# sloisel/MultiGridBarrier.jl

Measured on AMD Instinct MI355X. Metric: Newton iters/sec + wall-clock to converge, 2D P2 p-Laplace L=9, higher is better.
Workload: dtype f64

## Files before the change

### multigridbarrier.jl_amd/csrc/api.cpp

```cpp
#include <chrono>
#include <cmath>
#include <cstring>
#include <algorithm>
#include <limits>
#include <memory>
#include <string>

#include "interpolate.hpp"
#include "problem.hpp"

using namespace mgbhip;

mgbhip_problem* problem_create(mgbhip_ctx* ctx, const mgbhip_problem_desc* d, mgbhip_problem* share);
int core_run(mgbhip_problem* P, double* z, const double* c, const mgbhip_options* opt, mgbhip_core_result* res);
int matched_t_run(mgbhip_problem* P, const double* z, const double* c, double t_default, double* t_out);

#ifdef MGB_STEP_PROBE
namespace mgbhip { void mf_debug_probe(long long* out64); }
#endif

static thread_local std::string g_last_error;

struct DeviceGuard {
    int prev = -1, dev = -1;
// ... 165 lines not shown

int mgbhip_hessian_pattern(mgbhip_problem* P, int32_t level, int64_t* nnz, const int32_t** rowptr,
                           const int32_t** colidx) {
    MGB_API_BEGIN_ON(P)
    check_level(P, level);
    P->ensure_plan(level);
    if (nnz) *nnz = P->levels[level].nnz;
    if (rowptr) *rowptr = P->levels[level].hHptr.data();
    if (colidx) *colidx = P->levels[level].hHcol.data();
    return MGBHIP_OK;
    MGB_API_END
}

int mgbhip_solve(mgbhip_problem* P, int32_t level, const double* g, double* x) {
    MGB_API_BEGIN_ON(P)
    check_level(P, level);
    MGB_REQUIRE(g && x, "null argument");
    hipStream_t st = P->stream();
    const size_t m = (size_t)P->levels[level].m;
    P->d_g.upload(g, m, st);
    P->factor(level);
    P->trisolve(level, P->d_g.p, P->d_nv.p);
    int status = P->levels[level].solver.status(st);
    if (status != MGBHIP_OK && P->lu_fallback(level, P->d_g.p, P->d_nv.p)) status = MGBHIP_OK;
    P->d_nv.download(x, m, st);
    MGB_HIP_CHECK(hipStreamSynchronize(st));
    if (status != MGBHIP_OK) g_last_error = "Cholesky met a non-positive pivot";
    return status;
    MGB_API_END
}

int mgbhip_set_hessian(mgbhip_problem* P, int32_t level, const double* values) {
    MGB_API_BEGIN_ON(P)
    check_level(P, level);
    MGB_REQUIRE(values, "null argument");
    P->ensure_plan(level);
    mgbhip::Level& L = P->levels[level];
    MGB_REQUIRE(L.Hval.n >= (size_t)L.nnz, "this level keeps no CSR value array");
    L.Hval.upload(values, (size_t)L.nnz, P->stream());
    MGB_HIP_CHECK(hipStreamSynchronize(P->stream()));
    L.have_H = true;
    L.H_in_slab = false;
    L.factored = false;
    return MGBHIP_OK;
    MGB_API_END
}

int mgbhip_solve_newton(mgbhip_problem* P, int32_t level, const double* g, double* x, double* lambda2) {
    MGB_API_BEGIN_ON(P)
    check_level(P, level);
    MGB_REQUIRE(g && x, "null argument");
    hipStream_t st = P->stream();
    const size_t m = (size_t)P->levels[level].m;
    P->d_g.upload(g, m, st);
    P->factor(level, P->d_g.p);
    P->trisolve_carried(level, P->d_nv.p);
    int status = P->levels[level].solver.status(st);
    if (status != MGBHIP_OK && P->lu_fallback(level, P->d_g.p, P->d_nv.p)) status = MGBHIP_OK;
    P->d_nv.download(x, m, st);
    MGB_HIP_CHECK(hipStreamSynchronize(st));
    if (lambda2) {
        double acc = 0.0;
        for (size_t i = 0; i < m; ++i) acc += g[i] * x[i];
        *lambda2 = acc;
    }
    if (status != MGBHIP_OK) g_last_error = "Cholesky met a non-positive pivot";
    return status;
    MGB_API_END
}

int mgbhip_problem_set_sharding(mgbhip_problem* P, int32_t level, int64_t n_iface, const int32_t* iface_cols, const double* own_mask) {
    MGB_API_BEGIN_ON(P)
    check_level(P, level);
    mgbhip::Level& L = P->levels[level];
    MGB_REQUIRE(!L.solver.analyzed, "sharding must be set before the first solve of the level");
    MGB_REQUIRE(own_mask != nullptr && n_iface >= 0 && n_iface <= L.m && (n_iface == 0 || iface_cols), "bad sharding arguments");
    L.h_iface.assign(iface_cols, iface_cols + n_iface);
    for (int64_t i = 0; i < n_iface; ++i) {
        MGB_REQUIRE(L.h_iface[i] >= 0 && L.h_iface[i] < L.m, "interface column out of range");
        MGB_REQUIRE(i == 0 || L.h_iface[i] > L.h_iface[i - 1], "interface columns must be strictly increasing");
// ... 8 lines not shown

int mgbhip_problem_set_collective(mgbhip_problem* P, mgbhip_allreduce_fn fn, void* user, int32_t accepts_device_ptr) {
    MGB_API_BEGIN_ON(P)
    P->coll_fn = fn;
    P->coll_user = user;
    P->coll_device = accepts_device_ptr != 0;
    return MGBHIP_OK;
    MGB_API_END
}

int mgbhip_newton_direction(mgbhip_problem* P, int32_t level, const double* s, const double* c, const double* z0, double* x,
                            double* lambda2, int32_t* condensed) {
    MGB_API_BEGIN_ON(P)
    check_level(P, level);
    MGB_REQUIRE(s && c && z0 && x, "null argument");
    hipStream_t st = P->stream();
    const size_t m = (size_t)P->levels[level].m;
    stage_inputs(P, level, s, c, z0);
    P->eval_f1(level, P->d_x.p, P->d_z0.p, P->d_c.p, P->d_g.p);
    P->eval_f2(level, P->d_x.p, P->d_z0.p, P->d_c.p, false, P->d_g.p);
    if (condensed) *condensed = P->levels[level].H_condensed ? 1 : 0;
    P->factor(level, P->d_g.p);
    P->trisolve_carried(level, P->d_nv.p);
    const int status = P->levels[level].solver.status(st);
    P->d_nv.download(x, m, st);
    if (lambda2) {
        std::vector<double> g(m);
        P->d_g.download(g.data(), m, st);
        MGB_HIP_CHECK(hipStreamSynchronize(st));
        double acc = 0.0;
        for (size_t i = 0; i < m; ++i) acc += g[i] * x[i];
        *lambda2 = acc;
    }
    MGB_HIP_CHECK(hipStreamSynchronize(st));
    if (status != MGBHIP_OK) g_last_error = "Cholesky met a non-positive pivot";
    return status;
    MGB_API_END
}


static double* vec_scratch(mgbhip_ctx* c, int64_t len) {
    c->vscratch.ensure((size_t)reduce_scratch_doubles(len));
    c->vscal.ensure(8);
    return c->vscratch.p;
}
static void same_ctx(const mgbhip_vec* a, const mgbhip_vec* b) {
    MGB_REQUIRE(a && b, "null vector");
// ... 149 lines not shown
    P->touch();
    P->eval_f1(level, s->buf.p, z0->buf.p, c->buf.p, grad->buf.p);
    return MGBHIP_OK;
    MGB_API_END
}

int mgbhip_f2_d(mgbhip_problem* P, int32_t level, const mgbhip_vec* s, const mgbhip_vec* c, const mgbhip_vec* z0) {
    MGB_API_BEGIN_ON(P)
    check_closure_args(P, level, s, c, z0);
    P->touch();
    P->eval_f2(level, s->buf.p, z0->buf.p, c->buf.p);
    return MGBHIP_OK;
    MGB_API_END
}

int mgbhip_solve_d(mgbhip_problem* P, int32_t level, const mgbhip_vec* g, mgbhip_vec* x) {
    MGB_API_BEGIN_ON(P)
    check_level(P, level);
    MGB_REQUIRE(g && x && g->ctx == P->ctx && x->ctx == P->ctx, "bad vector");
    MGB_REQUIRE(g->len == P->levels[level].m && x->len == g->len, "solve: length mismatch");
    hipStream_t st = P->stream();
    P->factor(level);
    P->trisolve(level, g->buf.p, x->buf.p);
    const int status = P->levels[level].solver.status(st);
    if (status != MGBHIP_OK) g_last_error = "Cholesky met a non-positive pivot";
    return status;
    MGB_API_END
}

int mgbhip_prolong_add(mgbhip_problem* P, int32_t level, const mgbhip_vec* s, mgbhip_vec* z) {
    MGB_API_BEGIN_ON(P)
    check_level(P, level);
    MGB_REQUIRE(s && z && s->ctx == P->ctx && z->ctx == P->ctx, "bad vector");
    const Level& Lv = P->levels[level];
    MGB_REQUIRE(s->len == Lv.m && z->len == Lv.rows, "prolong_add: length mismatch");
    launch_csr_matvec(Lv.rows, Lv.Rptr.p, Lv.Rcol.p, Lv.Rval.p, s->buf.p, z->buf.p, true, false, P->stream());
    P->touch();
    return MGBHIP_OK;
    MGB_API_END
}

static int node_map(mgbhip_problem* P, const double* z, double* F, double* Dz, int mode) {
    MGB_REQUIRE(P && z && F, "null argument");
    hipStream_t st = P->stream();
    P->d_z0.upload(z, (size_t)P->nu * P->n, st);
    ElemParams E = P->base_params(-1, nullptr, P->d_z0.p, nullptr);
    if (Dz) {
// ... 168 lines not shown
```

### multigridbarrier.jl_amd/csrc/driver.cpp

```cpp
#include <chrono>
#include <cstdio>
#include <cstdlib>
#include <cmath>
#include <cstring>
#include <functional>
#include <limits>

#include "problem.hpp"

using namespace mgbhip;

namespace {

constexpr double EPS = std::numeric_limits<double>::epsilon();

bool debug_on() {
    static const bool on = [] { const char* e = getenv("MGBHIP_DEBUG"); return e && e[0] == '1'; }();
    return on;
}
#define DBG(...) do { if (debug_on()) { fprintf(stderr, __VA_ARGS__); } } while (0)

struct Stop {
    double lambda_tol;
    double theta;
// ... 162 lines not shown
    double y = C.F0(P->d_x.p);
    if (!std::isfinite(y)) throw InvalidArgument("newton: initial objective value is not finite");
    double ymin = y;
    if (P->sharded()) { P->d_gpart.ensure((size_t)C.m); P->d_gnpart.ensure((size_t)C.m); }
    C.F1(P->d_x.p, P->d_g.p, P->d_gpart.p);
    VecStats gs = vec_stats(P, C.level, P->d_g.p, C.m);
    if (gs.bad != 0.0 || !std::isfinite(gs.sumsq)) throw InvalidArgument("newton: initial gradient has non-finite entries");
    double gnorm = std::sqrt(gs.sumsq);
    double gmin = gnorm;
    double incmin = INFINITY;
    int k = 0;
    bool converged = false;
    Level& L = P->levels[C.level];
    struct RobustReset {
        MfSolver& s;
        ~RobustReset() { s.robust = false; }
    } robust_reset{L.solver};
    while (k < maxit && !converged) {
        ++k;
        C.F2(P->d_x.p);
        auto t0 = std::chrono::steady_clock::now();
        int fstatus = MGBHIP_OK;
        int leaf_flag = 0;
        for (int attempt = 0; attempt < 2; ++attempt) {
            P->factor(C.level, C.rhs_of_g());
            P->trisolve_carried(C.level, P->d_nv.p);
            const double seq = P->next_seq();
            launch_dir_finish(P->d_nv.p, P->d_g.p, C.m, P->d_scratch.p, P->d_scal.p, L.solver.status_flags_rw(), P->pin.dev, st,
                              P->own_mask(C.level), seq);
            L.solver.flags_cleared();
            P->wait_results(seq);
            P->pin.i[1] = P->pin.d[5] != 0.0 ? 1 : 0;
            leaf_flag |= P->pin.d[6] != 0.0 ? 1 : 0;
            P->pin.i[2] = leaf_flag;
            fstatus = MfSolver::status_from(P->pin.i + 1, L.solver.factored_condensed);
            if (P->sharded()) {
                P->pin.d[5] = fstatus != MGBHIP_OK ? 1.0 : 0.0;
                P->allreduce_host(P->pin.d + 2, 4, 0);
                fstatus = P->pin.d[5] != 0.0 ? MGBHIP_ERR_NOT_SPD : MGBHIP_OK;
            }
            const bool at_floor = std::fabs(P->pin.d[4]) <= EPS * std::fmax(std::fabs(y), 1.0);
            const bool suspicious = fstatus != MGBHIP_OK || P->pin.d[3] != 0.0 || !std::isfinite(P->pin.d[2]) ||
                                    (!(P->pin.d[4] > 0) && !at_floor);
            if (!suspicious || attempt == 1 || !L.solver.has_inverse_path() || L.solver.robust) break;
            DBG("newton[lev %d] k=%d: direction rejected (status %d, lambda^2=%.3e): refactoring with the substitution kernels\n",
                C.level, k, fstatus, P->pin.d[4]);
            L.solver.robust = true;
            L.factored = false;
        }
        if (fstatus != MGBHIP_OK && P->lu_fallback(C.level, P->d_g.p, P->d_nv.p)) {
            DBG("newton[lev %d] k=%d: LDL' met a zero pivot; direction from the pivoted LU fallback\n", C.level, k);
            launch_dir_finish(P->d_nv.p, P->d_g.p, C.m, P->d_scratch.p, P->d_scal.p, L.solver.status_flags_rw(), P->pin.dev, st,
                              P->own_mask(C.level));
            L.solver.flags_cleared();
            MGB_HIP_CHECK(hipStreamSynchronize(st));
            fstatus = MGBHIP_OK;
        }
// ... 231 lines not shown
    const bool sh = P->sharded();
    if (sh) { P->d_gpart.ensure((size_t)m); P->d_gnpart.ensure((size_t)m); }
    P->eval_f1(lev, P->d_x.p, P->d_z0.p, P->d_c.p, P->d_g.p, sh ? P->d_gpart.p : nullptr);
    P->eval_f1(lev, P->d_x.p, P->d_z0.p, P->d_c0.p, P->d_gn.p, sh ? P->d_gnpart.p : nullptr);
    launch_axpy(-1.0, P->d_g.p, P->d_gn.p, m, st);
    if (sh) launch_axpy(-1.0, P->d_gpart.p, P->d_gnpart.p, m, st);
    P->eval_f2(lev, P->d_x.p, P->d_z0.p, P->d_c0.p);
    if (sh) {
        P->d_tmp.ensure((size_t)m + 1);
        P->factor(lev, P->d_gpart.p);
        P->trisolve_carried(lev, P->d_tmp.p);
        int bad = P->levels[lev].solver.status(st) != MGBHIP_OK;
        MGB_HIP_CHECK(hipMemcpyAsync(P->d_nv.p, P->d_tmp.p, sizeof(double) * (size_t)m, hipMemcpyDeviceToDevice, st));
        P->levels[lev].factored = false;
        P->factor(lev, P->d_gnpart.p);
        P->trisolve_carried(lev, P->d_tmp.p);
        bad |= P->levels[lev].solver.status(st) != MGBHIP_OK;
        MGB_HIP_CHECK(hipMemcpyAsync(P->d_xn.p, P->d_tmp.p, sizeof(double) * (size_t)m, hipMemcpyDeviceToDevice, st));
        double fb = bad ? 1.0 : 0.0;
        P->allreduce_host(&fb, 1, 0);
        if (fb != 0.0) return MGBHIP_OK;
    } else {
        P->factor(lev);
        if (P->levels[lev].solver.status(st) != MGBHIP_OK) return MGBHIP_OK;
        P->trisolve(lev, P->d_g.p, P->d_nv.p);
        P->trisolve(lev, P->d_gn.p, P->d_xn.p);
    }
    const double d = dev_dot(P, lev, P->d_gn.p, P->d_xn.p, m);
    const double b = dev_dot(P, lev, P->d_g.p, P->d_xn.p, m) + dev_dot(P, lev, P->d_gn.p, P->d_nv.p, m);
    if (!(d > 0)) return MGBHIP_OK;
    const double tstar = -b / (2 * d);
    if (!(std::isfinite(tstar) && tstar > 0)) return MGBHIP_OK;
    *t_out = std::fmin(std::fmax(tstar, std::sqrt(EPS)), t_default);
    return MGBHIP_OK;
}
```

### multigridbarrier.jl_amd/csrc/mf_numeric.hip

```cpp
#include <hip/hip_runtime.h>

#include <cstdio>

#include <algorithm>
#include <cstdlib>

#include "../../include/mgbhip.h"
#include "mf_solver.hpp"

namespace mgbhip {

namespace {

#ifdef MGB_STEP_PROBE
__device__ long long g_probe[64];
#define SPL(i) do { if (threadIdx.x == 0 && gridDim.x == 1024 && blockIdx.x == 700 && j0 == 0) g_probe[48 + i] = wall_clock64(); } while (0)
#define SP(i) do { if (threadIdx.x == 0 && gridDim.x == 4096 && blockIdx.x == 3000) g_probe[40 + i] = wall_clock64(); if (threadIdx.x == 0 && gridDim.x == 1024 && blockIdx.x == 700) g_probe[24 + i] = wall_clock64(); } while (0)
#else
#define SPL(i) do { } while (0)
#define SP(i) do { } while (0)
#endif

typedef double double4_t __attribute__((ext_vector_type(4)));
constexpr int TX = 16;
// ... 1499 lines not shown
    PROBE(3);
    double4_t acc[4];
#pragma unroll
    for (int tb = 0; tb < 4; ++tb) acc[tb] = double4_t{0.0, 0.0, 0.0, 0.0};
#pragma unroll
    for (int kk = 0; kk < NB / 4; ++kk) {
        const double s = Pa[4 * kk + fk][16 * wave + fr16];
#pragma unroll
        for (int tb = 0; tb < 4; ++tb) {
            if (ti == tj && tb > wave) continue;
            acc[tb] = __builtin_amdgcn_mfma_f64_16x16x4f64(Pb[4 * kk + fk][16 * tb + fr16], s, acc[tb], 0, 0, 0);
        }
    }
    const int nskip = (blockIdx.x == 0 && look) ? nbn : 0;
#pragma unroll
    for (int tb = 0; tb < 4; ++tb)
#pragma unroll
        for (int r = 0; r < 4; ++r) {
            const int row = rbase + 16 * wave + fr16, col = cbase + 16 * tb + fk + 4 * r;
            if (row < m && col < m && row >= col && !(row - j1 < nskip && col - j1 < nskip))
                W[row + (int64_t)col * m] = cw[tb][r] - acc[tb][r];
        }
    PROBE(4);
}

__global__ __launch_bounds__(256) void mf_tri_pack(int m, const double* __restrict__ F, double* __restrict__ packed, int unpack,
                                                   double* __restrict__ Fout) {
    const int c = blockIdx.x;
    if (c >= m) return;
    const int64_t base = (int64_t)c * m - ((int64_t)c * (c - 1)) / 2;
    for (int r = c + threadIdx.x; r < m; r += 256) {
        if (unpack) Fout[r + (int64_t)c * m] = packed[base + (r - c)];
        else packed[base + (r - c)] = F[r + (int64_t)c * m];
    }
}

__global__ __launch_bounds__(256) void mf_big_diag0(const FrontDev* __restrict__ fr, int32_t first,
                                                    const double* __restrict__ arena, double* __restrict__ dscr,
                                                    int32_t* __restrict__ status) {
    __shared__ double Wv[NB][NB + 1];
    __shared__ double Dn[NB][NB + 1];
    __shared__ double Tm[16][17];
    __shared__ double dq[NB];
    const FrontDev F = fr[first + blockIdx.x];
    const int m = F.m, nb = min(NB, F.k), tid = threadIdx.x;
    const double* W = arena + F.F_off;
// ... 681 lines not shown
        d_a_dst.upload(ad, st);
        MGB_HIP_CHECK(hipStreamSynchronize(st));
        h_a_dst.swap(ad);
    }
    level_solves.assign(nlev, {});
    for (int32_t l = 0; l < nlev; ++l) {
        MfLaunch S{};
        for (auto& L : level_launches[l]) {
            if (!L.cls || L.tiny) { level_solves[l].push_back(L); continue; }
            if (S.count == 0) S = L;
            else {
                S.count += L.count;
                S.max_m = std::max(S.max_m, L.max_m);
                S.max_k = std::max(S.max_k, L.max_k);
            }
        }
        if (S.count) level_solves[l].insert(level_solves[l].begin(), S);
    }
    int32_t max_big = 1;
    for (auto& lev : level_launches)
        for (auto& L : lev)
            if (!L.cls) max_big = std::max(max_big, L.count);
    d_dscr.alloc((size_t)max_big * 2 * NB * NB);
    if (const char* e = getenv("MGBHIP_DEBUG"); e && atoi(e) >= 2) {
        fprintf(stderr, "[mgbhip] solver plan: n=%lld fronts=%d levels=%d arena=%.1f MB\n", (long long)plan.n, nf, nlev,
                plan.arena_doubles * 8e-6);
        for (int32_t l = 0; l < nlev; ++l)
            for (auto& L : level_launches[l]) {
                double sm = 0, sk = 0, fl = 0;
                for (int32_t q = L.first; q < L.first + L.count; ++q) {
                    const Front& f = plan.fronts[q];
                    sm += f.m; sk += f.k;
                    for (int c = 0; c < f.k; ++c) fl += (double)(f.m - c) * (f.m - c);
                }
                fprintf(stderr, "[mgbhip]   level %2d cls %3d count %7d max_m %4d max_k %4d avg_m %6.1f avg_k %6.1f Mflop %8.2f\n",
                        l, L.cls, L.count, L.max_m, L.max_k, sm / L.count, sk / L.count, fl * 1e-6);
            }
    }
    analyzed = true;
    MGB_HIP_CHECK(hipStreamSynchronize(st));
}


static StageTimers g_dummy_timers;
static StageTimers* timers_or_dummy(StageTimers* t, bool on) { return (t && on) ? t : &g_dummy_timers; }

bool MfSolver::launch_big_assemble(const MfLaunch& L, dim3 ga, const double* d_values, const int32_t* a_src_p, hipStream_t st,
                                   bool with_diag) {
    const size_t lds = (size_t)L.max_child * (size_t)L.max_m * sizeof(int32_t);
    if (L.max_child >= 1 && L.max_child <= GATHER_MAX_CHILD && lds <= 40 * 1024) {
        const int ct = CT;
        if (with_diag) ga.x += 1;
        hipLaunchKernelGGL(mf_big_gather, ga, dim3(256), lds, st, cur_fr, L.first, d_children.p, d_rel.p, a_src_p,
                           cur_adst, cur_acol, d_values, d_arena.p, L.max_m, d_dscr.p, d_status.p, with_diag ? 1 : 0, ct);
        return with_diag;
    } else
        hipLaunchKernelGGL(mf_big_assemble, ga, dim3(256), 0, st, cur_fr, L.first, d_children.p, d_rel.p, a_src_p,
                           cur_adst, cur_acol, d_values, d_arena.p);
    return false;
// ... 5 lines not shown
        const int64_t src = plan.a_src[t];
        const int64_t v = src < nnz ? (int64_t)value_map[src] : tail_base + (src - nnz);
        MGB_REQUIRE(v < (int64_t)INT32_MAX, "direct value index exceeds 32 bits");
        as[t] = (int32_t)v;
    }
    d_a_src_direct.upload(as, st);
    MGB_HIP_CHECK(hipStreamSynchronize(st));
}

void MfSolver::factor(const double* d_values, hipStream_t st, StageTimers* timers, bool direct, bool condensed) {
    MGB_REQUIRE(!direct || d_a_src_direct.n > 0, "MfSolver::factor: no direct value map");
    MGB_REQUIRE(!condensed || (direct && condensed_ok), "MfSolver::factor: condensed leaves are not enabled");
    const int32_t* a_src_p = condensed ? d_a_src_c.p : (direct ? d_a_src_direct.p : d_a_src.p);
    cur_fr = condensed ? d_fronts_c.p : d_fronts.p;
    cur_adst = condensed ? d_a_dst_c.p : d_a_dst.p;
    cur_acol = condensed ? d_a_colptr_c.p : d_a_colptr.p;
    MGB_REQUIRE(analyzed, "MfSolver::factor before analyze");
    if (timers) timers->begin("factor");
    factored_inv = !robust;
    if (!status_zero) MGB_HIP_CHECK(hipMemsetAsync(d_status.p, 0, sizeof(int32_t), st));
    status_zero = false;
    factored_condensed = condensed;
    static const bool lvl_timing = [] { const char* e = getenv("MGBHIP_LEVEL_TIMING"); return e && e[0] == '1'; }();
    int lvno = -1;
    for (auto& lev : level_launches) {
        ++lvno;
        char nm[32];
        snprintf(nm, sizeof(nm), "fac_lv%02d", lvno);
        StageScope lvscope(*timers_or_dummy(timers, lvl_timing), nm);
        for (auto& L : lev) {
            if (L.count == 0) continue;
            if (condensed && lvno == 0) continue;
            if (L.tiny) {
                hipLaunchKernelGGL(mf_factor_tiny, dim3((L.count + 15) / 16), dim3(256), 0, st, cur_fr, L.first,
                                   L.count, a_src_p, cur_adst, d_values, d_arena.p, d_status.p);
            } else if (L.wave) {
                const dim3 gw((L.count + 3) / 4);
                if (L.cls <= 32) {
                    const size_t lds = (size_t)4 * (32 * 33 / 2) * sizeof(double) + 4 * 64 * (sizeof(int64_t) + sizeof(int32_t));
                    hipLaunchKernelGGL(mf_factor_wave<32>, gw, dim3(256), lds, st, cur_fr, L.first, L.count, d_children.p, d_rel.p,
                                       a_src_p, cur_adst, d_values, d_arena.p, d_status.p);
                } else {
                    const size_t lds = (size_t)4 * (48 * 49 / 2) * sizeof(double) + 4 * 64 * (sizeof(int64_t) + sizeof(int32_t));
                    hipLaunchKernelGGL(mf_factor_wave<48>, gw, dim3(256), lds, st, cur_fr, L.first, L.count, d_children.p, d_rel.p,
                                       a_src_p, cur_adst, d_values, d_arena.p, d_status.p);
                }
// ... 21 lines not shown
                }
                if (L.inv && !robust) {
                    hipLaunchKernelGGL(mf_big_diag0, dim3(1), dim3(256), 0, st, cur_fr, L.first, d_arena.p, d_dscr.p, d_status.p);
                    for (int j0 = 0; j0 < L.max_k; j0 += NB) {
                        const int rem = L.max_m - j0;
                        const int T = std::max(0, (rem - 1 + ST - 1) / ST);
                        hipLaunchKernelGGL(mf_big_step, dim3(T * (T + 1) / 2 + 1, 1), dim3(256), 0, st, cur_fr, L.first, j0, d_arena.p,
                                           d_dscr.p, d_dvec.p, d_status.p, 0);
                    }
                } else {
                    for (int j0 = 0; j0 < L.max_k; j0 += NB) {
                        const int rem = L.max_m - j0;
                        hipLaunchKernelGGL(mf_big_panel, dim3(std::max(1, (rem - 1 + TR - 1) / TR), 1), dim3(256), 0, st, cur_fr,
                                           L.first, j0, d_arena.p, d_dscr.p, d_status.p, j0 == 0 ? 1 : 0);
                        const int T = (rem - 1 + ST - 1) / ST;
                        if (T > 0)
                            hipLaunchKernelGGL(mf_big_update, dim3(T * (T + 1) / 2 + 1, 1), dim3(256), 0, st, cur_fr, L.first, j0,
                                               d_arena.p, d_dscr.p, d_status.p);
                    }
                }
            } else if (L.inv && !robust) {
                const dim3 ga((L.max_m + CT - 1) / CT, L.count);
                const bool diag_done = launch_big_assemble(L, ga, d_values, a_src_p, st, true);
                const bool pre_diag = diag_done || L.count >= 24;
                if (pre_diag && !diag_done)
                    hipLaunchKernelGGL(mf_big_diag0, dim3(L.count), dim3(256), 0, st, cur_fr, L.first, d_arena.p, d_dscr.p,
                                       d_status.p);
                for (int j0 = 0; j0 < L.max_k; j0 += NB) {
                    const int rem = L.max_m - j0;
                    const int T = std::max(0, (rem - 1 + ST - 1) / ST);
                    const dim3 gs(T * (T + 1) / 2 + 1, L.count);
                    hipLaunchKernelGGL(mf_big_step, gs, dim3(256), 0, st, cur_fr, L.first, j0, d_arena.p, d_dscr.p,
                                       d_dvec.p, d_status.p, (j0 == 0 && !pre_diag) ? 1 : 0);
                }
            } else {
                const dim3 ga((L.max_m + CT - 1) / CT, L.count);
                launch_big_assemble(L, ga, d_values, a_src_p, st, false);
                for (int j0 = 0; j0 < L.max_k; j0 += NB) {
                    const int rem = L.max_m - j0;
                    const dim3 gp(std::max(1, (rem - 1 + TR - 1) / TR), L.count);
                    hipLaunchKernelGGL(mf_big_panel, gp, dim3(256), 0, st, cur_fr, L.first, j0, d_arena.p,
                                       d_dscr.p, d_status.p, j0 == 0 ? 1 : 0);
                    const int T = (rem - 1 + ST - 1) / ST;
                    if (T > 0) {
                        const dim3 gu(T * (T + 1) / 2 + 1, L.count);
                        hipLaunchKernelGGL(mf_big_update, gu, dim3(256), 0, st, cur_fr, L.first, j0, d_arena.p,
// ... 148 lines not shown
            for (int32_t q = L.first; q < L.first + L.count; ++q) {
                const Front& f = plan.fronts[q];
                const double mk = (double)(f.m - f.k), steps = (double)((f.k + NB - 1) / NB);
                extra += 2.0 * 0.5 * (mk * mk + mk * f.k) * std::max(0.0, steps - 1.0);
            }
        }
        if (lev_blocks) { big_levels += 1; blocks += lev_blocks; }
    }
    for (auto& lev : level_solves)
        for (auto& L : lev)
            if (L.count) bwd += 1;
    out[0] = blocks; out[1] = big_levels; out[2] = fac; out[3] = bwd;
    out[4] = (double)plan.arena_doubles; out[5] = (double)plan.factor_flops; out[6] = extra; out[7] = 0.0;
}

void MfSolver::status_async(int32_t* h_dst2, hipStream_t st) const {
    MGB_HIP_CHECK(hipMemcpyAsync(h_dst2, d_status.p, 2 * sizeof(int32_t), hipMemcpyDeviceToHost, st));
}

int MfSolver::status(hipStream_t st) {
    int32_t h[2] = {0, 0};
    d_status.download(h, 2, st);
    MGB_HIP_CHECK(hipStreamSynchronize(st));
    return status_from(h, factored_condensed);
}

bool MfSolver::enable_condensed(int64_t N, int P, const int32_t* ucol, int64_t slack0, int64_t nnz, int64_t tail_base,
                                hipStream_t st) {
    condensed_ok = false;
    int why = 0;
    struct Report { int& w; ~Report() { if (w) if (const char* e = getenv("MGBHIP_DEBUG"); e && atoi(e) >= 2) fprintf(stderr, "[mgbhip] condensed leaves: plan shape check %d failed\n", w); } } report{why};
    const int32_t nlev = (int32_t)plan.level_ptr.size() - 1;
    if (!analyzed || !plan.border || nlev < 2 || P > 7) { why = 1; return false; }
    const int32_t n0 = plan.level_ptr[1];
    if ((int64_t)n0 != N) { why = 2; return false; }
    const int32_t nbor = (int32_t)plan.n;
    std::vector<LeafDesc> desc((size_t)N);
    std::vector<char> seen((size_t)N, 0);
    for (int32_t i = 0; i < n0; ++i) {
        const Front& f = plan.fronts[i];
        const int32_t* idx = plan.front_idx.data() + f.idx_off;
        if (f.k != P + 1 || f.m > 15 || f.nchild != 0 || idx[f.m - 1] != nbor) { why = 3; return false; }
        const int64_t e = ((int64_t)idx[0] - slack0) / P;
        if (e < 0 || e >= N || seen[(size_t)e]) { why = 4; return false; }
        for (int q = 0; q < P; ++q)
            if ((int64_t)idx[q] != slack0 + e * P + q) { why = 5; return false; }
        if (idx[P] != ucol[e * P + (P - 1)] || idx[P] < 0) { why = 6; return false; }
// ... 53 lines not shown
```

### multigridbarrier.jl_amd/csrc/mf_solver.hpp

```cpp
#pragma once
#include <functional>

#include "common.hpp"
#include "mf_analysis.hpp"
#include "kernels.hpp"

namespace mgbhip {

struct FrontDev {
    int32_t k, m, nchild, a_cnt;
    int64_t F_off, idx_off, u_off, child_off, rel_off, a_off, acol_off;
    int64_t ug_off;
    int32_t packed;
    int32_t pad_;
};

struct MfLaunch {
    int32_t first, count;
    int32_t cls;
    int32_t max_m, max_k;
    int32_t max_child = 0;
    bool tiny = false;
    bool wave = false;
    bool inv = false;
    bool iface = false;
};

class MfSolver {
   public:
    MfPlan plan;
    void analyze(int64_t n, const int32_t* rowptr, const int32_t* colidx, hipStream_t st,
                 const double* coords = nullptr, int dim = 0, bool protect_peeled = false,
                 const int32_t* top = nullptr, int64_t ntop = 0);
    std::function<void(double*, int64_t)> iface_reduce;
    void factor(const double* d_values, hipStream_t st, StageTimers* timers, bool direct = false, bool condensed = false);
    bool enable_condensed(int64_t N, int P, const int32_t* ucol, int64_t slack0, int64_t nnz, int64_t tail_base, hipStream_t st);
    bool condensed_ready() const { return condensed_ok; }
    bool leaves_packed() const { return leaf_packed; }
    const LeafDesc* leaf_desc() const { return d_leaf_desc.p; }
    double* arena() { return d_arena.p; }
    int32_t* leaf_status() { return d_status.p + 1; }
    const int32_t* status_flags() const { return d_status.p; }
    int32_t* status_flags_rw() { return d_status.p; }
    void flags_cleared() { status_zero = true; leaf_zero = true; }
    bool leaf_flag_zero() const { return leaf_zero; }
    void leaf_flag_used() { leaf_zero = false; }
    void set_direct_map(const int32_t* value_map, int64_t nnz, int64_t tail_base, hipStream_t st);
    bool has_direct_map() const { return d_a_src_direct.n > 0; }
    void solve(const double* d_b, double* d_x, hipStream_t st, StageTimers* timers);
    void solve_border(double* d_x_np1, hipStream_t st, StageTimers* timers);
    void chain_stats(double* out8) const;
    int status(hipStream_t st);
    void status_async(int32_t* h_dst, hipStream_t st) const;
    static int status_from(const int32_t* flags2, bool with_leaves) {
        return (flags2[0] || (with_leaves && flags2[1])) ? MGBHIP_ERR_NOT_SPD : MGBHIP_OK;
    }
    bool factored_condensed = false;
    bool analyzed = false;
    bool robust = false;
    bool has_inverse_path() const { return uses_inv; }
    bool factored_inv = false;

   private:
    bool launch_big_assemble(const MfLaunch& L, dim3 grid, const double* d_values, const int32_t* a_src_p, hipStream_t st,
                             bool with_diag);
    void forward_pass(const double* d_b_np1, hipStream_t st, StageTimers* timers);
    void backward_pass(double* d_x_np1, hipStream_t st, StageTimers* timers);
    DevBuf<double> d_bx, d_xx, d_one;
    DevBuf<FrontDev> d_fronts;
    DevBuf<int32_t> d_front_idx, d_children, d_rel, d_a_src, d_a_src_direct, d_a_dst, d_a_colptr;
    DevBuf<int64_t> d_ug_ptr, d_ug_src;
    DevBuf<double> d_arena, d_uvec, d_y, d_tbig, d_tsol, d_dscr, d_dvec;
    DevBuf<double> d_ifpack;
    DevBuf<int32_t> d_status;
    bool condensed_ok = false;
    bool leaf_packed = false;
    std::vector<FrontDev> h_fronts;
    std::vector<int32_t> h_a_dst;
    DevBuf<FrontDev> d_fronts_c;
    DevBuf<int32_t> d_a_src_c, d_a_dst_c, d_a_colptr_c;
    DevBuf<LeafDesc> d_leaf_desc;
    const FrontDev* cur_fr = nullptr;
    const int32_t* cur_adst = nullptr;
    const int32_t* cur_acol = nullptr;
    std::vector<std::vector<MfLaunch>> level_launches;
    std::vector<std::vector<MfLaunch>> level_solves;
    int32_t lds_cap = 88;
    bool uses_inv = false;
    bool y_border_one = false;
    bool y_zero = false;
    bool status_zero = false, leaf_zero = false;
};

}
```

Baseline: 675.8.

## Fuse per-step big-front factor launches into one persistent level kernel with flag sync

Adds a persistent kernel that factors every big front in a tree level in a single launch. Lookahead workgroups produce the diagonal block inverses and tile workgroups apply the trailing updates, coordinated through epoch-tagged global flags with spin-waits. This removes the per-block-step kernel launches and the serialization between them. A timeout marks the factor as given up, and the caller then refactors with the old per-step launches, at the risk of deadlock-style stalls if the workgroups are not all co-resident, plus extra code complexity.

```diff
diff --git a/multigridbarrier.jl_amd/csrc/api.cpp b/multigridbarrier.jl_amd/csrc/api.cpp
--- a/multigridbarrier.jl_amd/csrc/api.cpp
+++ b/multigridbarrier.jl_amd/csrc/api.cpp
@@ -211,6 +211,11 @@
     P->factor(level);
     P->trisolve(level, P->d_g.p, P->d_nv.p);
     int status = P->levels[level].solver.status(st);
+    if (P->levels[level].solver.take_give_up()) {
+        P->factor(level);
+        P->trisolve(level, P->d_g.p, P->d_nv.p);
+        status = P->levels[level].solver.status(st);
+    }
     if (status != MGBHIP_OK && P->lu_fallback(level, P->d_g.p, P->d_nv.p)) status = MGBHIP_OK;
     P->d_nv.download(x, m, st);
     MGB_HIP_CHECK(hipStreamSynchronize(st));
@@ -245,6 +250,11 @@
     P->factor(level, P->d_g.p);
     P->trisolve_carried(level, P->d_nv.p);
     int status = P->levels[level].solver.status(st);
+    if (P->levels[level].solver.take_give_up()) {
+        P->factor(level, P->d_g.p);
+        P->trisolve_carried(level, P->d_nv.p);
+        status = P->levels[level].solver.status(st);
+    }
     if (status != MGBHIP_OK && P->lu_fallback(level, P->d_g.p, P->d_nv.p)) status = MGBHIP_OK;
     P->d_nv.download(x, m, st);
     MGB_HIP_CHECK(hipStreamSynchronize(st));
@@ -299,7 +309,12 @@
     if (condensed) *condensed = P->levels[level].H_condensed ? 1 : 0;
     P->factor(level, P->d_g.p);
     P->trisolve_carried(level, P->d_nv.p);
-    const int status = P->levels[level].solver.status(st);
+    int status = P->levels[level].solver.status(st);
+    if (P->levels[level].solver.take_give_up()) {
+        P->factor(level, P->d_g.p);
+        P->trisolve_carried(level, P->d_nv.p);
+        status = P->levels[level].solver.status(st);
+    }
     P->d_nv.download(x, m, st);
     if (lambda2) {
         std::vector<double> g(m);
@@ -495,7 +510,12 @@
     hipStream_t st = P->stream();
     P->factor(level);
     P->trisolve(level, g->buf.p, x->buf.p);
-    const int status = P->levels[level].solver.status(st);
+    int status = P->levels[level].solver.status(st);
+    if (P->levels[level].solver.take_give_up()) {
+        P->factor(level);
+        P->trisolve(level, g->buf.p, x->buf.p);
+        status = P->levels[level].solver.status(st);
+    }
     if (status != MGBHIP_OK) g_last_error = "Cholesky met a non-positive pivot";
     return status;
     MGB_API_END
diff --git a/multigridbarrier.jl_amd/csrc/driver.cpp b/multigridbarrier.jl_amd/csrc/driver.cpp
--- a/multigridbarrier.jl_amd/csrc/driver.cpp
+++ b/multigridbarrier.jl_amd/csrc/driver.cpp
@@ -208,6 +208,7 @@
         auto t0 = std::chrono::steady_clock::now();
         int fstatus = MGBHIP_OK;
         int leaf_flag = 0;
+        bool level_redo = false;
         for (int attempt = 0; attempt < 2; ++attempt) {
             P->factor(C.level, C.rhs_of_g());
             P->trisolve_carried(C.level, P->d_nv.p);
@@ -219,6 +220,14 @@
             P->pin.i[1] = P->pin.d[5] != 0.0 ? 1 : 0;
             leaf_flag |= P->pin.d[6] != 0.0 ? 1 : 0;
             P->pin.i[2] = leaf_flag;
+            if (!level_redo && L.solver.take_give_up((int32_t)P->pin.d[5])) {
+                DBG("newton[lev %d] k=%d: level kernel gave up a wait (%lld so far): refactoring with the per-step launches\n",
+                    C.level, k, (long long)L.solver.level_give_ups);
+                level_redo = true;
+                L.factored = false;
+                --attempt;
+                continue;
+            }
             fstatus = MfSolver::status_from(P->pin.i + 1, L.solver.factored_condensed);
             if (P->sharded()) {
                 P->pin.d[5] = fstatus != MGBHIP_OK ? 1.0 : 0.0;
@@ -496,7 +505,12 @@
         if (fb != 0.0) return MGBHIP_OK;
     } else {
         P->factor(lev);
-        if (P->levels[lev].solver.status(st) != MGBHIP_OK) return MGBHIP_OK;
+        int fst = P->levels[lev].solver.status(st);
+        if (P->levels[lev].solver.take_give_up()) {
+            P->factor(lev);
+            fst = P->levels[lev].solver.status(st);
+        }
+        if (fst != MGBHIP_OK) return MGBHIP_OK;
         P->trisolve(lev, P->d_g.p, P->d_nv.p);
         P->trisolve(lev, P->d_gn.p, P->d_xn.p);
     }
diff --git a/multigridbarrier.jl_amd/csrc/mf_numeric.hip b/multigridbarrier.jl_amd/csrc/mf_numeric.hip
--- a/multigridbarrier.jl_amd/csrc/mf_numeric.hip
+++ b/multigridbarrier.jl_amd/csrc/mf_numeric.hip
@@ -1545,6 +1545,309 @@
                 W[row + (int64_t)col * m] = cw[tb][r] - acc[tb][r];
         }
     PROBE(4);
+}
+
+typedef uint32_t __attribute__((address_space(1))) lv_gu32;
+typedef unsigned long long __attribute__((address_space(1))) lv_gu64;
+__device__ __forceinline__ double lv_ld(const double* p) {
+    return __longlong_as_double((long long)__hip_atomic_load((lv_gu64*)p, __ATOMIC_RELAXED, __HIP_MEMORY_SCOPE_AGENT));
+}
+__device__ __forceinline__ void lv_st(double* p, double v) {
+    __hip_atomic_store((lv_gu64*)p, (unsigned long long)__double_as_longlong(v), __ATOMIC_RELAXED, __HIP_MEMORY_SCOPE_AGENT);
+}
+
+struct LvFlags {
+    uint32_t* base;
+    int nblk, tm;
+    __device__ uint32_t* w(int b) const { return base + b; }
+    __device__ uint32_t* corner(int b) const { return base + nblk + b; }
+    __device__ uint32_t* col(int b, int I) const { return base + 2 * nblk + b * tm + I; }
+};
+
+__device__ __forceinline__ bool lv_acquire(uint32_t* const* fl, int n, uint32_t epoch, long long limit,
+                                           int32_t* status, int* s_ok, int tid) {
+    if (n == 0) return true;
+    if (tid < 64) {
+        bool ok = limit > 0;
+        const long long t0 = wall_clock64();
+        for (int i = 0; i < n && ok; ++i) {
+            while (__hip_atomic_load((lv_gu32*)fl[i], __ATOMIC_RELAXED, __HIP_MEMORY_SCOPE_AGENT) != epoch) {
+                if (wall_clock64() - t0 > limit) { ok = false; break; }
+                __builtin_amdgcn_s_sleep(1);
+            }
+        }
+        if (tid == 0) {
+            if (!ok) atomicOr(status, MF_LEVEL_GAVE_UP);
+            *s_ok = ok ? 1 : 0;
+        }
+    }
+    __syncthreads();
+    __builtin_amdgcn_fence(__ATOMIC_ACQUIRE, "wavefront");
+    const bool ok = *s_ok != 0;
+    __syncthreads();
+    return ok;
+}
+
+__device__ __forceinline__ void lv_publish(uint32_t* flag, uint32_t epoch, int tid) {
+    asm volatile("s_waitcnt vmcnt(0)" ::: "memory");
+    __syncthreads();
+    if (tid == 0) __hip_atomic_store((lv_gu32*)flag, epoch, __ATOMIC_RELAXED, __HIP_MEMORY_SCOPE_AGENT);
+}
+
+__device__ __forceinline__ void lv_write_mj(const double (*Wv)[NB + 1], const double* dq, double* W, double* dvec, int64_t idx_off,
+                                            int m, int j0, int nb, int lane, int wave) {
+    const int fr16 = lane & 15, fk = lane >> 4;
+    const int rt = wave & 1, ct = wave >> 1;
+    if (ct <= rt) {
+        double4_t accm = {0.0, 0.0, 0.0, 0.0};
+#pragma unroll
+        for (int kk = 0; kk < NB / 4; ++kk) {
+            const int kq = 4 * kk + fk;
+            accm = __builtin_amdgcn_mfma_f64_16x16x4f64(kq < nb ? Wv[kq][16 * ct + fr16] / dq[kq] : 0.0, Wv[kq][16 * rt + fr16], accm, 0, 0, 0);
+        }
+#pragma unroll
+        for (int r = 0; r < 4; ++r) {
+            const int row = 16 * rt + fr16, col = 16 * ct + fk + 4 * r;
+            if (row < nb && col < row) W[(j0 + col) + (int64_t)(j0 + row) * m] = accm[r];
+            else if (row < nb && col == row) dvec[idx_off + j0 + row] = accm[r];
+        }
+    }
+}
+
+__device__ __forceinline__ void lv_load_slot(const double* slot, double (*Wv)[NB + 1], double* dq, int nb, int tid) {
+    for (int i = tid; i < NB * NB; i += 256) {
+        const int rr = i % NB, c = i / NB;
+        const double v = (rr >= c && rr < nb) ? lv_ld(slot + rr + NB * c) : 0.0;
+        Wv[rr][c] = (rr > c) ? v : (rr == c ? 1.0 : 0.0);
+        if (rr == c) dq[rr] = (rr < nb) ? v : 1.0;
+    }
+}
+
+constexpr int LV_WAVES_PER_SIMD = 2;
+
+__global__ __launch_bounds__(256, LV_WAVES_PER_SIMD) void mf_big_step_level(
+        const FrontDev* __restrict__ fr, int32_t first, int32_t count, const int32_t* __restrict__ tile_pref,
+        double* __restrict__ arena, const double* __restrict__ dscr, double* __restrict__ lslot, double* __restrict__ dvec,
+        int32_t* __restrict__ status, uint32_t* __restrict__ flags, int nblkmax, int tmmax, uint32_t epoch, long long limit) {
+    __shared__ double Wv[NB][NB + 1];
+    __shared__ double Dn[NB][NB + 1];
+    __shared__ double Tm[16][17];
+    __shared__ double dq[NB], rdq[NB];
+    __shared__ double Pa[NB][ST + 1];
+    __shared__ double Pb[NB][ST + 1];
+    __shared__ int s_ok;
+    const int tid = threadIdx.x, lane = tid & 63, wave = tid >> 6;
+    const int fr16 = lane & 15, fk = lane >> 4;
+    const bool is_la = (int)blockIdx.x < count;
+    int f = 0, lin = 0;
+    if (is_la) {
+        f = blockIdx.x;
+    } else {
+        const int t = blockIdx.x - count;
+        while (f + 1 < count && tile_pref[f + 1] <= t) ++f;
+        lin = t - tile_pref[f];
+    }
+    const FrontDev F = fr[first + f];
+    const int m = F.m, k = F.k;
+    const int nblk = (k + NB - 1) / NB, Tmf = (m + ST - 1) / ST;
+    double* W = arena + F.F_off;
+    const LvFlags FL{flags + (int64_t)f * nblkmax * (2 + tmmax), nblkmax, tmmax};
+    double* myslots = lslot + (int64_t)f * nblkmax * (NB * NB);
+    const double* slot0 = dscr + (int64_t)f * 2 * (NB * NB);
+    uint32_t* wl[3];
+
+    if (is_la) {
+        lv_load_slot(slot0, Wv, dq, min(NB, k), tid);
+        for (int j = 0; j < nblk; ++j) {
+            const int j0 = j * NB, nb = min(NB, k - j0), j1 = j0 + nb;
+            const bool look = j1 < k;
+            const int nbn = look ? min(NB, k - j1) : 0;
+            __syncthreads();
+            if (tid < NB) rdq[tid] = 1.0 / dq[tid];
+            if ((j + 1) / 2 >= Tmf) lv_write_mj(Wv, dq, W, dvec, F.idx_off, m, j0, nb, lane, wave);
+            if (!look) break;
+            int nw = 0;
+            if (j >= 1) wl[nw++] = FL.col(j, (j + 1) / 2);
+            if (j + 1 >= 2) wl[nw++] = FL.corner(j + 1);
+            if (!lv_acquire(wl, nw, epoch, limit, status, &s_ok, tid)) return;
+            double pa[NB * ST / 256], cc[4];
+#pragma unroll
+            for (int u = 0; u < NB * ST / 256; ++u) {
+                const int i = tid + 256 * u, rr = i % ST, q = i / ST;
+                pa[u] = (q < nb && rr < nbn) ? lv_ld(W + (j1 + rr) + (int64_t)(j0 + q) * m) : 0.0;
+            }
+#pragma unroll
+            for (int t = 0; t < 4; ++t) {
+                const int i = tid + 256 * t, rr = i % NB, c = i / NB;
+                cc[t] = (rr >= c && rr < nbn) ? lv_ld(W + (j1 + rr) + (int64_t)(j1 + c) * m) : 0.0;
+            }
+#pragma unroll
+            for (int u = 0; u < NB * ST / 256; ++u) {
+                const int i = tid + 256 * u, rr = i % ST, q = i / ST;
+                Pa[q][rr] = pa[u];
+                Pb[q][rr] = 0.0;
+            }
+            __syncthreads();
+            if (wave < 2) slice_transform(Pa, Pa, Pb, Wv, rdq, lane, wave);
+            __syncthreads();
+            {
+                const int rt = wave & 1, ct = wave >> 1;
+                double4_t accd = {0.0, 0.0, 0.0, 0.0};
+#pragma unroll
+                for (int kk = 0; kk < NB / 4; ++kk)
+                    accd = __builtin_amdgcn_mfma_f64_16x16x4f64(Pb[4 * kk + fk][16 * ct + fr16], Pa[4 * kk + fk][16 * rt + fr16],
+                                                                accd, 0, 0, 0);
+#pragma unroll
+                for (int r = 0; r < 4; ++r) {
+                    const int rr = 16 * rt + fr16, c = 16 * ct + fk + 4 * r;
+                    Dn[rr][c] = -accd[r];
+                }
+            }
+            __syncthreads();
+#pragma unroll
+            for (int t = 0; t < 4; ++t) {
+                const int i = tid + 256 * t, rr = i % NB, c = i / NB;
+                Dn[rr][c] = (rr >= c && rr < nbn) ? cc[t] + Dn[rr][c] : 0.0;
+            }
+            __syncthreads();
+            block_ldlt32(Dn, dq, nbn, tid, status);
+            block_inverse32_sel(Dn, Wv, Tm, tid);
+            double* nslot = myslots + (int64_t)(j + 1) * (NB * NB);
+            for (int i = tid; i < NB * NB; i += 256) {
+                const int rr = i % NB, c = i / NB;
+                if (rr >= c && rr < nbn) lv_st(nslot + rr + NB * c, (rr == c) ? dq[rr] : Wv[rr][c]);
+            }
+            lv_publish(FL.w(j + 1), epoch, tid);
+            for (int i = tid; i < NB * NB; i += 256) {
+                const int rr = i % NB, c = i / NB;
+                if (rr == c) {
+                    if (rr >= nbn) dq[rr] = 1.0;
+                    Wv[rr][c] = 1.0;
+                } else if (rr < c || rr >= nbn) {
+                    Wv[rr][c] = 0.0;
+                }
+            }
+        }
+        return;
+    }
+
+    int I = (int)((sqrt(8.0 * lin + 1.0) - 1.0) * 0.5);
+    while ((I + 1) * (I + 2) / 2 <= lin) ++I;
+    while (I * (I + 1) / 2 > lin) --I;
+    const int J = lin - I * (I + 1) / 2;
+    const int r0 = ST * I, c0 = ST * J;
+    double cw[4][4];
+#pragma unroll
+    for (int tb = 0; tb < 4; ++tb)
+#pragma unroll
+        for (int r = 0; r < 4; ++r) {
+            const int row = r0 + 16 * wave + fr16, col = c0 + 16 * tb + fk + 4 * r;
+            cw[tb][r] = (row < m && col < m && row >= col) ? W[row + (int64_t)col * m] : 0.0;
+        }
+    const int jlast = min(2 * J + 1, nblk - 1);
+    for (int j = 0; j <= jlast; ++j) {
+        const int j0 = j * NB, nb = min(NB, k - j0), j1 = j0 + nb;
+        const bool mw = I == J && (j + 1) / 2 == J;
+        const bool work = c0 + ST - 1 >= j1 && m > j1;
+        if (!work && !mw) continue;
+        if (j >= 1) {
+            int nw = 0;
+            wl[nw++] = FL.w(j);
+            wl[nw++] = FL.col(j, I);
+            if (I != J) wl[nw++] = FL.col(j, J);
+            if (!lv_acquire(wl, nw, epoch, limit, status, &s_ok, tid)) return;
+        }
+        double pa[NB * ST / 256], pb[NB * ST / 256];
+#pragma unroll
+        for (int u = 0; u < NB * ST / 256; ++u) {
+            const int i = tid + 256 * u, rr = i % ST, q = i / ST;
+            const int r = r0 + rr, c = c0 + rr;
+            pa[u] = (q < nb && r >= j1 && r < m) ? lv_ld(W + r + (int64_t)(j0 + q) * m) : 0.0;
+            pb[u] = (I != J && q < nb && c >= j1 && c < m) ? lv_ld(W + c + (int64_t)(j0 + q) * m) : 0.0;
+        }
+        lv_load_slot(j == 0 ? slot0 : myslots + (int64_t)j * (NB * NB), Wv, dq, nb, tid);
+#pragma unroll
+        for (int u = 0; u < NB * ST / 256; ++u) {
+            const int i = tid + 256 * u, rr = i % ST, q = i / ST;
+            Pa[q][rr] = pa[u];
+            Pb[q][rr] = pb[u];
+        }
+        __syncthreads();
+        if (tid < NB) rdq[tid] = 1.0 / dq[tid];
+        if (mw) lv_write_mj(Wv, dq, W, dvec, F.idx_off, m, j0, nb, lane, wave);
+        __syncthreads();
+        if (work) {
+            if (I == J) {
+                slice_transform(Pa, Pa, Pb, Wv, rdq, lane, wave);
+            } else {
+                slice_transform(Pa, Pa, nullptr, Wv, rdq, lane, wave);
+                const int rr = 16 * wave + fr16;
+                double4_t acc0 = {0.0, 0.0, 0.0, 0.0}, acc1 = {0.0, 0.0, 0.0, 0.0};
+#pragma unroll
+                for (int kk = 0; kk < NB / 4; ++kk) {
+                    const double a = Pb[4 * kk + fk][rr];
+                    if (kk < 4) acc0 = __builtin_amdgcn_mfma_f64_16x16x4f64(Wv[fr16][4 * kk + fk], a, acc0, 0, 0, 0);
+                    acc1 = __builtin_amdgcn_mfma_f64_16x16x4f64(Wv[16 + fr16][4 * kk + fk], a, acc1, 0, 0, 0);
+                }
+#pragma unroll
+                for (int r = 0; r < 4; ++r) {
+                    const int q0 = fk + 4 * r, q1 = 16 + fk + 4 * r;
+                    Pb[q0][rr] = acc0[r] * rdq[q0];
+                    Pb[q1][rr] = acc1[r] * rdq[q1];
+                }
+            }
+            __syncthreads();
+            double4_t acc[4];
+#pragma unroll
+            for (int tb = 0; tb < 4; ++tb) acc[tb] = double4_t{0.0, 0.0, 0.0, 0.0};
+#pragma unroll
+            for (int kk = 0; kk < NB / 4; ++kk) {
+                const double s = Pa[4 * kk + fk][16 * wave + fr16];
+#pragma unroll
+                for (int tb = 0; tb < 4; ++tb) {
+                    if (I == J && tb > wave) continue;
+                    acc[tb] = __builtin_amdgcn_mfma_f64_16x16x4f64(Pb[4 * kk + fk][16 * tb + fr16], s, acc[tb], 0, 0, 0);
+                }
+            }
+#pragma unroll
+            for (int tb = 0; tb < 4; ++tb)
+#pragma unroll
+                for (int r = 0; r < 4; ++r) {
+                    const int row = r0 + 16 * wave + fr16, col = c0 + 16 * tb + fk + 4 * r;
+                    if (row >= j1 && col >= j1 && row < m && col < m && row >= col) cw[tb][r] = cw[tb][r] - acc[tb][r];
+                }
+        }
+        __syncthreads();
+        const bool pc = I == J && j + 2 < nblk && (j + 2) / 2 == J;
+        const bool pp = j + 1 < nblk && (j + 1) / 2 == J;
+        if (pc || pp) {
+            const int cb0 = (j + 2) * NB, cnb = pc ? min(NB, k - cb0) : 0;
+            const int pb0 = (j + 1) * NB, pnb = pp ? min(NB, k - pb0) : 0;
+#pragma unroll
+            for (int tb = 0; tb < 4; ++tb)
+#pragma unroll
+                for (int r = 0; r < 4; ++r) {
+                    const int row = r0 + 16 * wave + fr16, col = c0 + 16 * tb + fk + 4 * r;
+                    const bool sc = row >= col && row >= cb0 && row < cb0 + cnb && col >= cb0 && col < cb0 + cnb;
+                    const bool sp = pp && col >= pb0 && col < pb0 + NB && row < m && col < m && row >= col &&
+                                    !(row >= pb0 && row < pb0 + pnb && col < pb0 + pnb);
+                    if (sc || sp) lv_st(W + row + (int64_t)col * m, cw[tb][r]);
+                }
+            asm volatile("s_waitcnt vmcnt(0)" ::: "memory");
+            __syncthreads();
+            if (tid == 0) {
+                if (pc) __hip_atomic_store((lv_gu32*)FL.corner(j + 2), epoch, __ATOMIC_RELAXED, __HIP_MEMORY_SCOPE_AGENT);
+                if (pp) __hip_atomic_store((lv_gu32*)FL.col(j + 1, I), epoch, __ATOMIC_RELAXED, __HIP_MEMORY_SCOPE_AGENT);
+            }
+        }
+    }
+#pragma unroll
+    for (int tb = 0; tb < 4; ++tb)
+#pragma unroll
+        for (int r = 0; r < 4; ++r) {
+            const int row = r0 + 16 * wave + fr16, col = c0 + 16 * tb + fk + 4 * r;
+            if (col >= k && row < m && col < m && row >= col) W[row + (int64_t)col * m] = cw[tb][r];
+        }
 }
 
 __global__ __launch_bounds__(256) void mf_tri_pack(int m, const double* __restrict__ F, double* __restrict__ packed, int unpack,
@@ -2272,6 +2575,47 @@
         for (auto& L : lev)
             if (!L.cls) max_big = std::max(max_big, L.count);
     d_dscr.alloc((size_t)max_big * 2 * NB * NB);
+    {
+        static const int lv_cap = [] {
+            constexpr int blocks_per_cu = LV_WAVES_PER_SIMD;
+            int dev = 0, cus = 256;
+            if (hipGetDevice(&dev) == hipSuccess) (void)hipDeviceGetAttribute(&cus, hipDeviceAttributeMultiprocessorCount, dev);
+            return std::max(1, cus) * (blocks_per_cu - 1);
+        }();
+        std::vector<int32_t> pref;
+        int64_t nflags = 0, nslot = 0;
+        for (auto& lev : level_launches)
+            for (auto& L : lev) {
+                L.lv_wgs = 0;
+                if (L.cls || L.tiny || L.wave || L.iface || !L.inv || L.count == 0) continue;
+                const size_t lds = (size_t)L.max_child * (size_t)L.max_m * sizeof(int32_t);
+                if (!(L.max_child >= 1 && L.max_child <= GATHER_MAX_CHILD && lds <= 40 * 1024)) continue;
+                int64_t wgs = L.count, nblk = 0, tm = 0;
+                std::vector<int32_t> p(1, 0);
+                for (int32_t q = L.first; q < L.first + L.count; ++q) {
+                    const Front& f = plan.fronts[q];
+                    const int64_t t = (f.m + ST - 1) / ST;
+                    wgs += t * (t + 1) / 2;
+                    p.push_back(p.back() + (int32_t)(t * (t + 1) / 2));
+                    nblk = std::max<int64_t>(nblk, (f.k + NB - 1) / NB);
+                    tm = std::max(tm, t);
+                }
+                if (wgs > lv_cap || nblk < 2) continue;
+                L.lv_wgs = (int32_t)wgs;
+                L.lv_pref = (int32_t)pref.size();
+                pref.insert(pref.end(), p.begin(), p.end());
+                L.lv_nblk = (int32_t)nblk;
+                L.lv_tm = (int32_t)tm;
+                L.lv_flags = nflags;
+                nflags += (int64_t)L.count * nblk * (2 + tm);
+                nslot = std::max(nslot, (int64_t)L.count * nblk * NB * NB);
+            }
+        d_lv_pref.upload(pref, st);
+        d_lv_flags.alloc((size_t)std::max<int64_t>(nflags, 4));
+        MGB_HIP_CHECK(hipMemsetAsync(d_lv_flags.p, 0, d_lv_flags.n * sizeof(uint32_t), st));
+        d_lv_slot.alloc((size_t)std::max<int64_t>(nslot, 1));
+        lv_epoch = 0;
+    }
     if (const char* e = getenv("MGBHIP_DEBUG"); e && atoi(e) >= 2) {
         fprintf(stderr, "[mgbhip] solver plan: n=%lld fronts=%d levels=%d arena=%.1f MB\n", (long long)plan.n, nf, nlev,
                 plan.arena_doubles * 8e-6);
@@ -2283,8 +2627,8 @@
                     sm += f.m; sk += f.k;
                     for (int c = 0; c < f.k; ++c) fl += (double)(f.m - c) * (f.m - c);
                 }
-                fprintf(stderr, "[mgbhip]   level %2d cls %3d count %7d max_m %4d max_k %4d avg_m %6.1f avg_k %6.1f Mflop %8.2f\n",
-                        l, L.cls, L.count, L.max_m, L.max_k, sm / L.count, sk / L.count, fl * 1e-6);
+                fprintf(stderr, "[mgbhip]   level %2d cls %3d count %7d max_m %4d max_k %4d avg_m %6.1f avg_k %6.1f Mflop %8.2f"
+                        " level-kernel WGs %d\n", l, L.cls, L.count, L.max_m, L.max_k, sm / L.count, sk / L.count, fl * 1e-6, L.lv_wgs);
             }
     }
     analyzed = true;
@@ -2336,6 +2680,20 @@
     status_zero = false;
     factored_condensed = condensed;
     static const bool lvl_timing = [] { const char* e = getenv("MGBHIP_LEVEL_TIMING"); return e && e[0] == '1'; }();
+    static const bool level_kernel = [] { const char* e = getenv("MGBHIP_NO_LEVEL_KERNEL"); return !(e && e[0] == '1'); }();
+    static const long long lv_limit = [] {
+        const char* e = getenv("MGBHIP_LEVEL_SPIN_US");
+        const long long us = e ? atoll(e) : 10000ll;
+        int dev = 0, khz = 100000;
+        if (hipGetDevice(&dev) == hipSuccess) (void)hipDeviceGetAttribute(&khz, hipDeviceAttributeWallClockRate, dev);
+        return std::max(0ll, us) * (long long)std::max(1, khz) / 1000ll;
+    }();
+    const bool use_level = level_kernel && !lv_off_once && !iface_reduce;
+    lv_off_once = false;
+    if (use_level && ++lv_epoch == 0) {
+        MGB_HIP_CHECK(hipMemsetAsync(d_lv_flags.p, 0, d_lv_flags.n * sizeof(uint32_t), st));
+        lv_epoch = 1;
+    }
     int lvno = -1;
     for (auto& lev : level_launches) {
         ++lvno;
@@ -2403,6 +2761,12 @@
             } else if (L.inv && !robust) {
                 const dim3 ga((L.max_m + CT - 1) / CT, L.count);
                 const bool diag_done = launch_big_assemble(L, ga, d_values, a_src_p, st, true);
+                if (diag_done && L.lv_wgs > 0 && use_level) {
+                    hipLaunchKernelGGL(mf_big_step_level, dim3(L.lv_wgs), dim3(256), 0, st, cur_fr, L.first, L.count,
+                                       d_lv_pref.p + L.lv_pref, d_arena.p, d_dscr.p, d_lv_slot.p, d_dvec.p, d_status.p,
+                                       d_lv_flags.p + L.lv_flags, L.lv_nblk, L.lv_tm, lv_epoch, lv_limit);
+                    continue;
+                }
                 const bool pre_diag = diag_done || L.count >= 24;
                 if (pre_diag && !diag_done)
                     hipLaunchKernelGGL(mf_big_diag0, dim3(L.count), dim3(256), 0, st, cur_fr, L.first, d_arena.p, d_dscr.p,
@@ -2597,7 +2961,18 @@
     int32_t h[2] = {0, 0};
     d_status.download(h, 2, st);
     MGB_HIP_CHECK(hipStreamSynchronize(st));
+    gave_up_seen = (h[0] & MF_LEVEL_GAVE_UP) != 0;
     return status_from(h, factored_condensed);
+}
+
+bool MfSolver::take_give_up(int32_t flag0) {
+    if (!(flag0 & MF_LEVEL_GAVE_UP)) return false;
+    ++level_give_ups;
+    lv_off_once = true;
+    if (const char* e = getenv("MGBHIP_DEBUG"); e && e[0] >= '1')
+        fprintf(stderr, "[mgbhip] level kernel gave up a wait (%lld so far): factoring once more with the per-step launches\n",
+                (long long)level_give_ups);
+    return true;
 }
 
 bool MfSolver::enable_condensed(int64_t N, int P, const int32_t* ucol, int64_t slack0, int64_t nnz, int64_t tail_base,
diff --git a/multigridbarrier.jl_amd/csrc/mf_solver.hpp b/multigridbarrier.jl_amd/csrc/mf_solver.hpp
--- a/multigridbarrier.jl_amd/csrc/mf_solver.hpp
+++ b/multigridbarrier.jl_amd/csrc/mf_solver.hpp
@@ -24,7 +24,13 @@
     bool wave = false;
     bool inv = false;
     bool iface = false;
+    int32_t lv_wgs = 0;
+    int32_t lv_pref = 0;
+    int32_t lv_nblk = 0, lv_tm = 0;
+    int64_t lv_flags = 0;
 };
+
+constexpr int32_t MF_LEVEL_GAVE_UP = 2;
 
 class MfSolver {
    public:
@@ -60,6 +66,9 @@
     bool robust = false;
     bool has_inverse_path() const { return uses_inv; }
     bool factored_inv = false;
+    bool take_give_up(int32_t flag0);
+    bool take_give_up() { const bool g = gave_up_seen; gave_up_seen = false; return g && take_give_up(MF_LEVEL_GAVE_UP); }
+    int64_t level_give_ups = 0;
 
    private:
     bool launch_big_assemble(const MfLaunch& L, dim3 grid, const double* d_values, const int32_t* a_src_p, hipStream_t st,
@@ -73,6 +82,12 @@
     DevBuf<double> d_arena, d_uvec, d_y, d_tbig, d_tsol, d_dscr, d_dvec;
     DevBuf<double> d_ifpack;
     DevBuf<int32_t> d_status;
+    DevBuf<int32_t> d_lv_pref;
+    DevBuf<uint32_t> d_lv_flags;
+    DevBuf<double> d_lv_slot;
+    uint32_t lv_epoch = 0;
+    bool lv_off_once = false;
+    bool gave_up_seen = false;
     bool condensed_ok = false;
     bool leaf_packed = false;
     std::vector<FrontDev> h_fronts;
```

New measurement: 687.2 (median of 6 runs). 1.7% higher.
